# theislab/dca

Hardware: AMD Instinct MI355X
Metric: cells/sec training (ZINB AE, 68k x 20k) (higher is better)
Workload: dtype f32

## Files before the change

### dca_amd/csrc/dcahip_heads.hip

```cpp
#include <hip/hip_runtime.h>
#include <stdint.h>
#include <type_traits>
#include "dcahip.h"
#include "zinb_math.hpp"

namespace {

using f32x16 = __attribute__((ext_vector_type(16))) float;

constexpr int kTG = 32;
constexpr int kTR = 32;
constexpr int kLdS = 33;
constexpr int kWG = 2;
constexpr int kMaxGrid = 2048;
constexpr int kMaxSmallGrid = 8192;
constexpr int kCUs = 256;
constexpr int kZU = 4;
constexpr int kQCap = 320;

__device__ __forceinline__ int rowmap(int e, int hi) { return (e & 3) + 8 * (e >> 2) + 4 * hi; }

__device__ __forceinline__ void wave_sync() {
    __builtin_amdgcn_fence(__ATOMIC_RELEASE, "wavefront");
    __builtin_amdgcn_wave_barrier();
    __builtin_amdgcn_fence(__ATOMIC_ACQUIRE, "wavefront");
}

using f16x8 = __attribute__((ext_vector_type(8))) _Float16;
using f16x2v = __attribute__((ext_vector_type(2))) _Float16;
using f32x2v = __attribute__((ext_vector_type(2))) float;
using u32x4 = __attribute__((ext_vector_type(4))) unsigned;
using u32x2 = __attribute__((ext_vector_type(2))) unsigned;
using s16x4 = __attribute__((ext_vector_type(4))) short;

constexpr int kWR2 = 8;
constexpr int kWr8MinNT = 5;
constexpr int kHTile = 2 * 32 * 64;
constexpr int kTop = 13;
constexpr int kDExp0 = 8;
constexpr float kDLim = 30000.f;
constexpr int kDSlack = 2;
constexpr int kEHZero = 64;

#define MFMAH(a, b, c) __builtin_amdgcn_mfma_f32_32x32x16_f16(__builtin_bit_cast(f16x8, a), __builtin_bit_cast(f16x8, b), c, 0, 0, 0)

__device__ __forceinline__ unsigned pk_f16(float a, float b) {
    return __builtin_bit_cast(unsigned, __builtin_convertvector(f32x2v{a, b}, f16x2v));
}
__device__ __forceinline__ float resid_lo(unsigned p, float x) {
    float r;
    asm("v_fma_mix_f32 %0, %1, -1.0, %2 op_sel:[0,0,0] op_sel_hi:[1,0,0]" : "=v"(r) : "v"(p), "v"(x));
    return r;
}
__device__ __forceinline__ float resid_hi(unsigned p, float x) {
    float r;
    asm("v_fma_mix_f32 %0, %1, -1.0, %2 op_sel:[1,0,0] op_sel_hi:[1,0,0]" : "=v"(r) : "v"(p), "v"(x));
    return r;
}
__device__ __forceinline__ void split_pair(float x0, float x1, unsigned& p0, unsigned& p1) {
    p0 = pk_f16(x0, x1);
    p1 = pk_f16(resid_lo(p0, x0), resid_hi(p0, x1));
}
__device__ __forceinline__ void split8(const float (&x)[8], u32x4 (&f)[2]) {
#pragma unroll
    for (int j = 0; j < 4; ++j) {
        unsigned a, b;
        split_pair(x[2 * j], x[2 * j + 1], a, b);
        f[0][j] = a; f[1][j] = b;
    }
}
#ifdef DCA_EXP_H2_TWO
#define MFMA_H3(A, Bf, ACC) { ACC = MFMAH(A[0], Bf[1], ACC); ACC = MFMAH(A[0], Bf[0], ACC); }
#else
#define MFMA_H3(A, Bf, ACC) { ACC = MFMAH(A[1], Bf[0], ACC); ACC = MFMAH(A[0], Bf[1], ACC); ACC = MFMAH(A[0], Bf[0], ACC); }
#endif

__device__ __forceinline__ float pow2i(int e) { return __uint_as_float((unsigned)(127 + e) << 23); }
__device__ __forceinline__ int block_exp(float m) {
    if (!(m > 0.f) || !(m < INFINITY)) return 0;
    const int e = kTop + 1 - __builtin_amdgcn_frexp_expf(m);
    return e < -60 ? -60 : (e > 60 ? 60 : e);
}
__device__ __forceinline__ float wave_max(float v) {
    int l = (int)__builtin_amdgcn_mbcnt_hi(~0u, __builtin_amdgcn_mbcnt_lo(~0u, 0u));
    asm volatile("" : "+v"(l));
#pragma unroll
    for (int off = 32; off > 0; off >>= 1)
        v = fmaxf(v, __int_as_float(__builtin_amdgcn_ds_bpermute((l ^ off) << 2, __float_as_int(v))));
    return v;
}

struct HeadsArgs2 {
    const unsigned short* HA;
    const unsigned short* HT;
    const int* eH;
    const float* H; long ldh;
    float* gW; long ldg;
    float* g_theta;
    const float* Wh; long ldw;
    const float* bh;
    const float* theta_w;
    const float* y;  long ldy;
    const unsigned char* yc; long ldc;
    const int* ovf_ptr; const int* ovf_col; const float* ovf_val;
    const float* sf;
    const int* perm;
    const long long* cursor;
    float* ws_dw;  long dw_stride;
    float* ws_dh;
    int npart, nitems;
    const int* tile_order;
    double* partials;
    long plane, ldws;
    int B, hL, G;
    int S, NT;
    float ridge, inv_n;
    int d_exp;
    int tile_base;
};

__device__ __forceinline__ float escaped_count(const HeadsArgs2& p, long srow, int col) {
    float v = 255.f;
    if (p.ovf_ptr)
        for (int i = p.ovf_ptr[srow], e = p.ovf_ptr[srow + 1]; i < e; ++i)
            if (p.ovf_col[i] == col) { v = p.ovf_val[i]; break; }
    return v;
}

__global__ __launch_bounds__(256) void heads_split_h_kernel(const float* H, long ldh, int B, int hL,
                                                            unsigned short* HA, unsigned short* HT, int* eH) {
    __shared__ unsigned short tr[2][64][32 + 2];
    __shared__ float wm[4];
    const int t = blockIdx.x, tid = threadIdx.x;
    const int row = tid >> 3, k0 = (tid & 7) * 8;
    const long grow = (long)t * 32 + row;
    float x[8];
    float m = 0.f;
#pragma unroll
    for (int j = 0; j < 8; ++j) {
        x[j] = (grow < B && k0 + j < hL) ? H[grow * ldh + k0 + j] : 0.f;
        m = fmaxf(m, fabsf(x[j]));
    }
    m = wave_max(m);
    if ((tid & 63) == 0) wm[tid >> 6] = m;
    __syncthreads();
    const int e = block_exp(fmaxf(fmaxf(wm[0], wm[1]), fmaxf(wm[2], wm[3])));
    if (tid == 0) eH[t] = (fmaxf(fmaxf(wm[0], wm[1]), fmaxf(wm[2], wm[3])) > 0.f) ? e : kEHZero;
    const float sc = pow2i(e);
#pragma unroll
    for (int j = 0; j < 8; ++j) x[j] *= sc;
    u32x4 f[2];
    split8(x, f);
    const int pos = (row & 0x13) | ((row & 4) << 1) | ((row & 8) >> 1);
#pragma unroll
    for (int q = 0; q < 2; ++q) {
        *reinterpret_cast<u32x4*>(HA + (((long)t * 2 + q) * 32 + row) * 64 + k0) = f[q];
#pragma unroll
        for (int j = 0; j < 8; ++j) tr[q][k0 + j][pos] = (unsigned short)(f[q][j >> 1] >> (16 * (j & 1)));
    }
    __syncthreads();
    for (int c = tid; c < 2 * 64 * 4; c += 256) {
        const int q = c >> 8, i = (c >> 2) & 63, part = c & 3;
        u32x4 v;
#pragma unroll
        for (int j = 0; j < 4; ++j) v[j] = (unsigned)tr[q][i][part * 8 + 2 * j] | ((unsigned)tr[q][i][part * 8 + 2 * j + 1] << 16);
        *reinterpret_cast<u32x4*>(HT + (((long)t * 2 + q) * 64 + i) * 32 + part * 8) = v;
    }
}

template <bool HAS_PI, bool CONST_DISP, bool YC>
__global__ __launch_bounds__(64 * kWR2) void heads_fused_h2_kernel(HeadsArgs2 p) {
    using YV = std::conditional_t<YC, unsigned, float>;
    constexpr int WR = kWR2;
    constexpr int NH = 1 + (CONST_DISP ? 0 : 1) + (HAS_PI ? 1 : 0);
    constexpr int PI_H = NH - 1;
    constexpr int KT = 64;
    constexpr int ST_PLANE = kTG * kLdS;
    constexpr int QCAP = 192;
    constexpr int CELL_LD = 144;
    constexpr int HEAD_B = kTG * CELL_LD;
    constexpr int ROWT = 96;
    constexpr int PW_FLOATS = NH * HEAD_B / 4 + (CONST_DISP ? ST_PLANE : 0) + QCAP * 4 + ROWT;
    constexpr int NTHREADS = 64 * WR;
    constexpr int W_PIECE = 64 * 64;
    constexpr int W_FLOATS = NH * 2 * W_PIECE / 4;
    constexpr int NRED = NH * 2 * 16 + NH + 1;
    constexpr int BIAS_FLOATS = (NH + 1) * 32;
    constexpr int LDS_FLOATS = W_FLOATS + WR * PW_FLOATS + BIAS_FLOATS;
    static_assert((WR / 2) * NRED * 64 <= LDS_FLOATS, "dW reduce scratch");
    __shared__ __attribute__((aligned(16))) float lds[LDS_FLOATS];
    __shared__ double lred[WR];
    __shared__ float wmaxs[WR];

    const int tid = threadIdx.x, lane = tid & 63;
    const int wave = __builtin_amdgcn_readfirstlane(tid >> 6);
    const int l31 = lane & 31, hi = lane >> 5;
    const int r = wave;
    const long long cur = p.cursor ? *p.cursor : 0;
    double dacc = 0.0;
    bool first_item = true;
    const int s_wg = blockIdx.x % p.S, wq = blockIdx.x / p.S;
    const int ngb = p.nitems / p.S;
    const int full = ngb / p.npart, rem = ngb - full * p.npart;
    const int nrounds = full + ((rem > 0 && ((full & 1) ? p.npart - 1 - wq : wq) < rem) ? 1 : 0);
    const int kD0 = kDExp0 + p.d_exp;
    int eHmin = 1 << 20;
    for (int t = s_wg * WR + r; t < p.NT; t += p.S * WR) { const int e = p.eH[t]; eHmin = (e != kEHZero && e < eHmin) ? e : eHmin; }
    eHmin = __builtin_amdgcn_readfirstlane(eHmin == (1 << 20) ? 0 : eHmin);
#pragma unroll 1
    for (int j = 0; j < nrounds; ++j) {
    const int gb = j * p.npart + ((j & 1) ? p.npart - 1 - wq : wq);
    int s_opaque = s_wg;
    asm volatile("" : "+v"(s_opaque));
    const int s = __builtin_amdgcn_readfirstlane(s_opaque);
    const int gt = p.tile_order ? p.tile_order[gb + p.tile_base] : gb + p.tile_base;
    const int g0 = gt * kTG;
    const int gene = g0 + l31;
    const bool tile_ok = g0 < p.G;
    const bool gvalid = gene < p.G;

    unsigned char* const Wimg = reinterpret_cast<unsigned char*>(lds);
    unsigned char* const Pimg = reinterpret_cast<unsigned char*>(lds + W_FLOATS + wave * PW_FLOATS);
    float* const Th = lds + W_FLOATS + wave * PW_FLOATS + NH * HEAD_B / 4;
    u32x4* const Qe = reinterpret_cast<u32x4*>(lds + W_FLOATS + wave * PW_FLOATS + NH * HEAD_B / 4 + (CONST_DISP ? ST_PLANE : 0));
    float* const Bs = lds + W_FLOATS + WR * PW_FLOATS;
    int* const Rt = reinterpret_cast<int*>(lds + W_FLOATS + wave * PW_FLOATS + PW_FLOATS - ROWT);
    float* const Sft = reinterpret_cast<float*>(Rt + 64);

    int eW = 0;
    if (tile_ok) {
        constexpr int UNR = (NH * 64 * 8 + NTHREADS - 1) / NTHREADS;
        constexpr int ITEMS = NH * 64 * 8;
        float4 v[UNR];
        float m = 0.f;
#pragma unroll
        for (int u = 0; u < UNR; ++u) {
            const int idx = tid + u * NTHREADS;
            const int c4 = idx & 7, kq = (idx >> 3) & 63, h = (idx >> 9) < NH ? (idx >> 9) : NH - 1;
            const int kc = kq < p.hL ? kq : p.hL - 1;
            long gcol = g0 + c4 * 4;
            if (gcol > p.plane - 4) gcol = p.plane - 4;
            v[u] = *reinterpret_cast<const float4*>(p.Wh + (long)kc * p.ldw + (long)h * p.plane + gcol);
        }
#pragma unroll
        for (int u = 0; u < UNR; ++u) {
            const int idx = tid + u * NTHREADS;
            const int c4 = idx & 7, kq = (idx >> 3) & 63;
            const int gcol = g0 + c4 * 4;
            const bool kv = idx < ITEMS && kq < p.hL && gcol <= p.plane - 4;
            if (!kv || gcol + 0 >= p.G) v[u].x = 0.f;
            if (!kv || gcol + 1 >= p.G) v[u].y = 0.f;
            if (!kv || gcol + 2 >= p.G) v[u].z = 0.f;
            if (!kv || gcol + 3 >= p.G) v[u].w = 0.f;
            m = fmaxf(fmaxf(m, fmaxf(fabsf(v[u].x), fabsf(v[u].y))), fmaxf(fabsf(v[u].z), fabsf(v[u].w)));
        }
        m = wave_max(m);
        if (lane == 0) wmaxs[wave] = m;
        __syncthreads();
        m = fmaxf(fmaxf(fmaxf(wmaxs[0], wmaxs[1]), fmaxf(wmaxs[2], wmaxs[3])), fmaxf(fmaxf(wmaxs[4], wmaxs[5]), fmaxf(wmaxs[6], wmaxs[7])));
        eW = __builtin_amdgcn_readfirstlane(block_exp(m));
        const float wsc = pow2i(eW);
#pragma unroll
        for (int u = 0; u < UNR; ++u) {
            const int idx = tid + u * NTHREADS;
            if (idx >= ITEMS) continue;
            const int c4 = idx & 7, kq = (idx >> 3) & 63, h = idx >> 9;
            unsigned a0, a1, b0, b1;
            split_pair(v[u].x * wsc, v[u].y * wsc, a0, a1);
            split_pair(v[u].z * wsc, v[u].w * wsc, b0, b1);
            const int off = kq * 64 + ((((c4 >> 1) + (kq >> 2)) & 3) << 4) + ((c4 & 1) << 3);
            *reinterpret_cast<u32x2*>(Wimg + (h * 2 + 0) * W_PIECE + off) = u32x2{a0, b0};
            *reinterpret_cast<u32x2*>(Wimg + (h * 2 + 1) * W_PIECE + off) = u32x2{a1, b1};
        }
        if (tid < 32) {
            const bool gv = g0 + tid < p.G;
#pragma unroll
            for (int h = 0; h < NH; ++h) Bs[h * 32 + tid] = gv ? p.bh[(long)h * p.plane + g0 + tid] : 0.f;
            Bs[NH * 32 + tid] = (CONST_DISP && gv) ? p.theta_w[g0 + tid] : 0.f;
        }
    }
    __syncthreads();

    f32x16 dW[NH][2];
#pragma unroll
    for (int h = 0; h < NH; ++h)
#pragma unroll
        for (int ib = 0; ib < 2; ++ib)
#pragma unroll
            for (int e = 0; e < 16; ++e) dW[h][ib][e] = 0.f;
    float bsum[NH];
#pragma unroll
    for (int h = 0; h < NH; ++h) bsum[h] = 0.f;
    float thsum = 0.f;

    if (tile_ok) {
        const int gene_c = gvalid ? gene : p.G - 1;
        const float* const ycol = p.y + gene_c;
        const unsigned char* const ycolc = p.yc + gene_c;
        const unsigned ldy_u = YC ? (unsigned)p.ldc : (unsigned)p.ldy;
        auto count_at = [&](int sr) -> YV {
            if constexpr (YC) return (unsigned)ycolc[(unsigned long long)(unsigned)sr * ldy_u];
            else return ycol[(unsigned long long)(unsigned)sr * ldy_u];
        };
        const int tstep = p.S * WR;
        int t = s * WR + r;
        const long dh_tstride = (long)p.npart * (kTR * KT);
        float* const dh_part = p.ws_dh + (long)(blockIdx.x / p.S) * (kTR * KT);
        const int dh_lane = ((((l31 & 0x13) | ((l31 & 4) << 1) | ((l31 & 8) >> 1)) * KT) + 4 * hi) * 4;
        int srow_l = 0;
        float sf_l = 1.f;
        YV yA[kZU], yB[kZU];
        auto row_clamped = [&](int tt) { const int rl = tt * kTR + l31; return rl < p.B ? rl : p.B - 1; };
        auto load_srow = [&](int tt) { const int rlc = row_clamped(tt); return p.perm ? p.perm[cur + rlc] : (int)(cur + rlc); };
        const __amdgpu_buffer_rsrc_t ha_rs = __builtin_amdgcn_make_buffer_rsrc(
            const_cast<unsigned short*>(p.HA), 0, p.NT * (kHTile * 2), 0x00020000);
        const __amdgpu_buffer_rsrc_t ht_rs = __builtin_amdgcn_make_buffer_rsrc(
            const_cast<unsigned short*>(p.HT), 0, p.NT * (kHTile * 2), 0x00020000);
        const int ha_lane = l31 * 128 + hi * 64;
        const int ht_lane = l31 * 64 + hi * 16;
        u32x4 ha0[2];
        auto load_ha = [&](int tt, int ks, u32x4 (&dst)[2]) {
            const int so = tt * (kHTile * 2);
            int ha_o = ha_lane;
            asm volatile("" : "+v"(ha_o));
#pragma unroll
            for (int q = 0; q < 2; ++q)
                dst[q] = __builtin_bit_cast(u32x4, __builtin_amdgcn_raw_buffer_load_b128(ha_rs, ha_o + q * 4096 + ks * 16, so, 0));
        };
        auto load_ht = [&](int tt, int ks, u32x4 (&dst)[2][2]) {
            const int so = tt * (kHTile * 2);
            int ht_o = ht_lane;
            asm volatile("" : "+v"(ht_o));
#pragma unroll
            for (int q = 0; q < 2; ++q)
#pragma unroll
                for (int ib = 0; ib < 2; ++ib)
                    dst[q][ib] = __builtin_bit_cast(u32x4, __builtin_amdgcn_raw_buffer_load_b128(
                        ht_rs, ht_o + q * 4096 + ib * 2048 + ks * 32, so, 0));
        };
        const int t16 = lane & 15, c8 = 4 * ((lane >> 4) & 1) + (t16 & 3);
        int wtr[4];
#pragma unroll
        for (int rr = 0; rr < 4; ++rr)
            wtr[rr] = hi * 2048 + (t16 >> 2) * 64 + ((((c8 >> 1) + rr) & 3) << 4) + ((c8 & 1) << 3);
        int wdr[2];
#pragma unroll
        for (int gs = 0; gs < 2; ++gs) wdr[gs] = l31 * 64 + (((2 * gs + hi + (l31 >> 2)) & 3) << 4);
        auto w_tr = [&](int h, int q, int ks) {
            const unsigned char* b0 = Wimg + (h * 2 + q) * W_PIECE + ks * 512;
            const s16x4 lo = __builtin_amdgcn_ds_read_tr16_b64_v4i16(
                (__attribute__((address_space(3))) s16x4*)(b0 + wtr[(2 * ks) & 3]));
            const s16x4 hi4 = __builtin_amdgcn_ds_read_tr16_b64_v4i16(
                (__attribute__((address_space(3))) s16x4*)(b0 + 256 + wtr[(2 * ks + 1) & 3]));
            u32x4 o;
            const u32x2 a = __builtin_bit_cast(u32x2, lo), b = __builtin_bit_cast(u32x2, hi4);
            o[0] = a[0]; o[1] = a[1]; o[2] = b[0]; o[3] = b[1];
            return o;
        };
        auto w_dr = [&](int h, int q, int jb, int gs) {
            return *reinterpret_cast<const u32x4*>(Wimg + (h * 2 + q) * W_PIECE + jb * 2048 + wdr[gs]);
        };
        const int cell_lane = l31 * CELL_LD + 2 * hi * 16;
        const int dtr = (8 * hi + (t16 >> 2)) * CELL_LD + c8 * 16;

        int eHt = 0;
        if (t < p.NT) {
            srow_l = load_srow(t);
            sf_l = p.sf[srow_l];
            eHt = p.eH[t];
            load_ha(t, 0, ha0);
            if (lane < 32) { Rt[l31] = srow_l; Sft[l31] = sf_l; }
            wave_sync();
            {
                const int4 r4 = *reinterpret_cast<const int4*>(Rt + 4 * hi);
                yA[0] = count_at(r4.x); yA[1] = count_at(r4.y); yA[2] = count_at(r4.z); yA[3] = count_at(r4.w);
            }
        }
        int rb = 0;
        int accE = eHmin + kD0;
        int tile_no = wave >> 2;
        for (; t < p.NT; t += tstep) {
            if ((tile_no++) & 1) __builtin_amdgcn_s_setprio(1); else __builtin_amdgcn_s_setprio(0);
            const int row0 = t * kTR;
            const int tn = t + tstep < p.NT ? t + tstep : t;
            eHt = __builtin_amdgcn_readfirstlane(eHt);
            const bool hzero = eHt == kEHZero;
            if (hzero) eHt = 0;
            const int kDa = accE - eHt;
            const int kDt = (!hzero && kDa <= kD0 && kDa >= kD0 - kDSlack) ? kDa : kD0;
            const float fscale = pow2i(eHt + eW), funscale = pow2i(-(eHt + eW));
            int kDe = kDt;
            float lacc;
            const float thw = CONST_DISP ? Bs[NH * 32 + l31] : 0.f;
            const int srow_n = load_srow(tn);
            if (lane < 32) Rt[(rb ^ 1) * 32 + l31] = srow_n;
            const int eHn = p.eH[tn];
            float scs = 0.f;
            int qn = 0;
            float dmax = 0.f;
            auto z_sparse = [&](int q0, int cnt) {
                const bool act = lane < cnt;
                const u32x4 ent = Qe[q0 + (act ? lane : 0)];
                const unsigned e = ent[0];
                const int gq = (e >> 5) & 31, row = e & 31;
                const float sfr = __shfl(sf_l, row, 64);
                const int sr = __shfl(srow_l, row, 64);
                const float am = __uint_as_float(ent[1]);
                const float ad = CONST_DISP ? Bs[NH * 32 + gq] : __uint_as_float(ent[2]);
                const float ap = HAS_PI ? __uint_as_float(ent[3]) : 0.f;
                float yq = (float)(e >> 16);
                if (__ballot(act && (e >> 16) == 0xFFFFu)) {
                    if (act && (e >> 16) == 0xFFFFu) yq = YC ? escaped_count(p, sr, g0 + gq) : p.y[(long)sr * p.ldy + g0 + gq];
                    __builtin_amdgcn_s_waitcnt(0x0F70);
                }
                float o[3] = {0.f, 0.f, 0.f};
                float nll;
                if (HAS_PI) {
                    nll = zinb_nz_elem<CONST_DISP, YC>(am, ad, ap, sfr, yq, p.ridge, o[0], o[1], o[2]);
                } else {
                    float dmu = 0.f, dth = 0.f, dpi = 0.f;
                    const Heads hd = head_acts<HAS_PI, CONST_DISP>(am, ad, ap, sfr);
                    nll = nll_elem<HAS_PI, true, true, YC>(hd, yq, p.ridge, dmu, dth, dpi);
                    o[0] = dmu * hd.gm; o[1] = dth * hd.gd;
                }
                lacc += act ? nll : 0.f;
                o[0] *= scs; o[1] *= scs; o[2] *= scs;
                dmax = fmaxf(dmax, act ? fmaxf(fmaxf(fabsf(o[0]), CONST_DISP ? 0.f : fabsf(o[1])), fabsf(o[2])) : 0.f);
                if (act) {
                    const int pos = (row & 0x13) | ((row & 4) << 1) | ((row & 8) >> 1);
                    unsigned char* pa = Pimg + gq * CELL_LD + (pos >> 2) * 16 + (pos & 3) * 2;
                    auto put = [&](int h, float v) {
                        const _Float16 h1 = (_Float16)v;
                        const _Float16 h2 = (_Float16)(v - (float)h1);
                        *reinterpret_cast<_Float16*>(pa + h * HEAD_B) = h1;
                        *reinterpret_cast<_Float16*>(pa + h * HEAD_B + 8) = h2;
                    };
                    put(0, o[0]);
                    if (CONST_DISP) Th[gq * kLdS + row] = o[1]; else put(1, o[1]);
                    if (HAS_PI) put(PI_H, o[2]);
                }
            };
            auto z_flush = [&](bool last) {
                while (qn >= 64 || (last && qn > 0)) {
                    const int c = qn < 64 ? qn : 64;
                    wave_sync();
                    z_sparse(qn - c, c);
                    qn -= c;
                }
            };
            auto z_dense = [&](auto fullv, int grp, const YV (&yv)[kZU]) {
                constexpr bool FULLV = decltype(fullv)::value;
                unsigned char* const cell = Pimg + cell_lane + ((grp & 1) + 4 * (grp >> 1)) * 16;
                float i_am[kZU], i_ad[kZU], i_ap[kZU];
                {
                    const float4 vm = *reinterpret_cast<const float4*>(cell);
                    i_am[0] = vm.x; i_am[1] = vm.y; i_am[2] = vm.z; i_am[3] = vm.w;
                    if (CONST_DISP) {
#pragma unroll
                        for (int j = 0; j < kZU; ++j) i_ad[j] = thw;
                    } else {
                        const float4 vd = *reinterpret_cast<const float4*>(cell + HEAD_B);
                        i_ad[0] = vd.x; i_ad[1] = vd.y; i_ad[2] = vd.z; i_ad[3] = vd.w;
                    }
                    if (HAS_PI) {
                        const float4 vp = *reinterpret_cast<const float4*>(cell + PI_H * HEAD_B);
                        i_ap[0] = vp.x; i_ap[1] = vp.y; i_ap[2] = vp.z; i_ap[3] = vp.w;
                    } else {
#pragma unroll
                        for (int j = 0; j < kZU; ++j) i_ap[j] = 0.f;
                    }
                }
                float o_m[kZU], o_d[kZU], o_p[kZU];
                bool o_nz[kZU];
                const float4 sf4 = *reinterpret_cast<const float4*>(Sft + 8 * grp + 4 * hi);
                const float sfj[kZU] = {sf4.x, sf4.y, sf4.z, sf4.w};
#pragma unroll
                for (int j = 0; j < kZU; ++j) {
                    const int row = rowmap(grp * kZU + j, hi);
                    const bool valid = FULLV || ((row0 + row < p.B) && gvalid);
                    const YV yj = yv[j];
                    bool nz;
                    if constexpr (YC) nz = valid && yj != 0u;
                    else nz = valid && (HAS_PI ? !(yj < kZeroThresh) : (yj != 0.f));
                    const float sc = (valid && !nz) ? scs : 0.f;
                    if (HAS_PI) {
                        float gmv, gdv, gpv;
                        const float nll = zinb_zero_elem<CONST_DISP>(i_am[j], i_ad[j], i_ap[j], sfj[j], p.ridge, gmv, gdv, gpv);
                        lacc += (valid && !nz) ? nll : 0.f;
                        o_m[j] = gmv * sc;
                        o_d[j] = gdv * sc;
                        o_p[j] = gpv * sc;
                        dmax = fmaxf(dmax, fmaxf(fabsf(o_m[j]), fabsf(o_p[j])));
                    } else {
                        float gmv, gdv;
                        const float nll = nb_zero_elem<CONST_DISP>(i_am[j], i_ad[j], sfj[j], gmv, gdv);
                        lacc += (valid && !nz) ? nll : 0.f;
                        o_m[j] = gmv * sc;
                        o_d[j] = gdv * sc;
                        o_p[j] = 0.f;
                        dmax = fmaxf(dmax, fabsf(o_m[j]));
                    }
                    if (!CONST_DISP) dmax = fmaxf(dmax, fabsf(o_d[j]));
                    o_nz[j] = nz;
                }
                {
                    auto put4 = [&](int h, const float (&v)[kZU]) {
                        unsigned a0, a1, b0, b1;
                        split_pair(v[0], v[1], a0, a1);
                        split_pair(v[2], v[3], b0, b1);
                        *reinterpret_cast<u32x4*>(cell + h * HEAD_B) = u32x4{a0, b0, a1, b1};
                    };
                    put4(0, o_m);
                    if (!CONST_DISP) put4(1, o_d);
                    if (HAS_PI) put4(PI_H, o_p);
                }
#pragma unroll
                for (int j = 0; j < kZU; ++j) {
                    const int row = rowmap(grp * kZU + j, hi);
                    const bool nz = o_nz[j];
                    const unsigned long long m = __ballot(nz);
                    const int slot = qn + __builtin_amdgcn_mbcnt_hi((unsigned)(m >> 32), __builtin_amdgcn_mbcnt_lo((unsigned)m, 0u));
                    if (nz) {
                        const YV yj = yv[j];
                        unsigned y16;
                        if constexpr (YC) y16 = yj == 255u ? 0xFFFFu : yj;
                        else y16 = (yj < 65535.f && yj == floorf(yj)) ? (unsigned)yj : 0xFFFFu;
                        Qe[slot] = u32x4{(unsigned)(l31 * 32 + row) | (y16 << 16), __float_as_uint(i_am[j]), __float_as_uint(i_ad[j]),
                                         __float_as_uint(i_ap[j])};
                    } else if (CONST_DISP) {
                        Th[l31 * kLdS + row] = o_d[j];
                    }
                    qn += __popcll(m);
                    if (j == 1) z_flush(false);
                }
                z_flush(false);
            };
            auto load_y = [&](int half, int grp, YV (&yv)[kZU]) {
                const int4 r4 = *reinterpret_cast<const int4*>(Rt + (rb ^ half) * 32 + 8 * grp + 4 * hi);
                yv[0] = count_at(r4.x); yv[1] = count_at(r4.y); yv[2] = count_at(r4.z); yv[3] = count_at(r4.w);
            };
            u32x4 htb[2][2][2];
            auto z_loop = [&](auto fullv) {
#pragma unroll 1
                for (int grp = 0; grp < 16 / kZU; ++grp) {
                    if (grp + 1 < 16 / kZU) load_y(0, grp + 1, yB);
                    else load_y(1, 0, yB);
                    z_dense(fullv, grp, yA);
#pragma unroll
                    for (int j = 0; j < kZU; ++j) yA[j] = yB[j];
                }
                load_ht(t, 0, htb[0]);
                __builtin_amdgcn_sched_barrier(0);
                z_flush(true);
            };
            for (;;) {
            f32x16 acc[NH];
#pragma unroll
            for (int h = 0; h < NH; ++h) {
                const float bias_h = Bs[h * 32 + l31] * fscale;
#pragma unroll
                for (int e = 0; e < 16; ++e) acc[h][e] = bias_h;
            }
            {
                u32x4 hb[2][2];
#pragma unroll
                for (int q = 0; q < 2; ++q) hb[0][q] = ha0[q];
#pragma unroll
                for (int ks = 0; ks < 4; ++ks) {
                    if (ks < 3) load_ha(t, ks + 1, hb[(ks + 1) & 1]);
                    __builtin_amdgcn_sched_barrier(0);
#pragma unroll
                    for (int h = 0; h < NH; ++h) {
                        u32x4 bf[2] = {w_tr(h, 0, ks), w_tr(h, 1, ks)};
                        MFMA_H3(hb[ks & 1], bf, acc[h])
                    }
                }
            }
#pragma unroll
            for (int h = 0; h < NH; ++h)
#pragma unroll
                for (int g = 0; g < 4; ++g)
                    *reinterpret_cast<float4*>(Pimg + h * HEAD_B + cell_lane + ((g & 1) + 4 * (g >> 1)) * 16) =
                        make_float4(acc[h][4 * g] * funscale, acc[h][4 * g + 1] * funscale, acc[h][4 * g + 2] * funscale, acc[h][4 * g + 3] * funscale);
            wave_sync();

            scs = pow2i(kDe);
            lacc = 0.f;
            qn = 0;
            dmax = 0.f;
            if (row0 + kTR <= p.B && g0 + kTG <= p.G) z_loop(std::true_type{}); else z_loop(std::false_type{});
            if (!__ballot(!(dmax <= kDLim))) break;
            const float mx = wave_max(dmax);
            const int need = __builtin_amdgcn_readfirstlane(__builtin_amdgcn_frexp_expf(mx) - 1 - kTop);
            if (!(need > 0) || kDe < kDt - 200) break;
            kDe -= need > 100 ? 100 : need;
            load_y(0, 0, yA);
            load_ha(t, 0, ha0);
            wave_sync();
            }
            dacc += (double)lacc;
            const float sf_n = p.sf[srow_n];
            wave_sync();
            if (!hzero && accE != eHt + kDe) {
                const int mv = eHt + kDe - accE;
                accE = eHt + kDe;
#pragma unroll
                for (int h = 0; h < NH; ++h)
#pragma unroll
                    for (int ib = 0; ib < 2; ++ib)
#pragma unroll
                        for (int e = 0; e < 16; ++e) dW[h][ib][e] = __builtin_amdgcn_ldexpf(dW[h][ib][e], mv);
            }

            const __amdgpu_buffer_rsrc_t dh_rs = __builtin_amdgcn_make_buffer_rsrc(
                dh_part + (long)t * dh_tstride, 0, kTR * KT * 4, 0x00020000);
            const __amdgpu_buffer_rsrc_t dh_rq = __builtin_amdgcn_make_buffer_rsrc(
                dh_part + (long)t * dh_tstride, 0, first_item ? 0 : kTR * KT * 4, 0x00020000);
            f32x16 dHa[2];
            int dh_o = dh_lane;
            asm volatile("" : "+v"(dh_o));
            load_ht(t, 1, htb[1]);
#pragma unroll
            for (int jb = 0; jb < 2; ++jb)
#pragma unroll
                for (int eq = 0; eq < 4; ++eq) {
                    const u32x4 u = __builtin_bit_cast(u32x4, __builtin_amdgcn_raw_buffer_load_b128(dh_rq, dh_o + 128 * jb + 32 * eq, 0, 0));
#pragma unroll
                    for (int w = 0; w < 4; ++w) { const unsigned uw = u[w]; dHa[jb][4 * eq + w] = __uint_as_float(uw); }
                }
            __builtin_amdgcn_sched_barrier(0);
            float tsum[NH];
#pragma unroll
            for (int h = 0; h < NH; ++h) tsum[h] = 0.f;
#pragma unroll
            for (int ks = 0; ks < 2; ++ks)
#pragma unroll
                for (int h = 0; h < NH; ++h) {
                    u32x4 bf[2];
#pragma unroll
                    for (int q = 0; q < 2; ++q) {
                        const unsigned char* c0 = Pimg + h * HEAD_B + cell_lane + 4 * ks * 16 + 8 * q;
                        const u32x2 lo = *reinterpret_cast<const u32x2*>(c0), hi2 = *reinterpret_cast<const u32x2*>(c0 + 16);
                        bf[q] = u32x4{lo[0], lo[1], hi2[0], hi2[1]};
#pragma unroll
                        for (int w = 0; w < 4; ++w) {
                            const unsigned pw = bf[q][w];
                            tsum[h] = __builtin_amdgcn_fdot2(__builtin_bit_cast(f16x2v, pw), f16x2v{(_Float16)1.f, (_Float16)1.f}, tsum[h], false);
                        }
                    }
#pragma unroll
                    for (int ib = 0; ib < 2; ++ib) {
                        u32x4 af[2] = {htb[ks][0][ib], htb[ks][1][ib]};
                        MFMA_H3(af, bf, dW[h][ib])
                    }
                }
#pragma unroll
            for (int h = 0; h < NH; ++h) asm volatile("" : "+v"(tsum[h]));
            {
                const float gun = pow2i(-kDe);
#pragma unroll
                for (int h = 0; h < NH; ++h) bsum[h] = fmaf(tsum[h], gun, bsum[h]);
                if (CONST_DISP) {
                    float ts = 0.f;
#pragma unroll
                    for (int e = 0; e < 16; ++e) ts += Th[l31 * kLdS + rowmap(e, hi)];
                    thsum = fmaf(ts, gun, thsum);
                }
            }
            load_ha(tn, 0, ha0);
            __builtin_amdgcn_sched_barrier(0);
            {
                const float fs = pow2i(kDe + eW), fu = pow2i(-(kDe + eW));
#pragma unroll
                for (int jb = 0; jb < 2; ++jb)
#pragma unroll
                    for (int e = 0; e < 16; ++e) {
                        float x = dHa[jb][e];
                        asm("v_mul_f32 %0, %1, %0" : "+v"(x) : "s"(fs));
                        dHa[jb][e] = x;
                    }
#pragma unroll
                for (int h = 0; h < NH; ++h)
#pragma unroll
                    for (int gs = 0; gs < 2; ++gs) {
                        u32x4 af[2];
#pragma unroll
                        for (int q = 0; q < 2; ++q) {
                            const unsigned char* b0 = Pimg + h * HEAD_B + gs * 16 * CELL_LD + 8 * q + dtr;
                            const s16x4 lo = __builtin_amdgcn_ds_read_tr16_b64_v4i16((__attribute__((address_space(3))) s16x4*)(b0));
                            const s16x4 hi4 = __builtin_amdgcn_ds_read_tr16_b64_v4i16((__attribute__((address_space(3))) s16x4*)(b0 + 4 * CELL_LD));
                            const u32x2 a = __builtin_bit_cast(u32x2, lo), b = __builtin_bit_cast(u32x2, hi4);
                            af[q] = u32x4{a[0], a[1], b[0], b[1]};
                        }
#pragma unroll
                        for (int jb = 0; jb < 2; ++jb) {
                            u32x4 bf[2] = {w_dr(h, 0, jb, gs), w_dr(h, 1, jb, gs)};
                            MFMA_H3(bf, af, dHa[jb])
                        }
                    }
#pragma unroll
                for (int jb = 0; jb < 2; ++jb)
#pragma unroll
                    for (int eq = 0; eq < 4; ++eq) {
                        u32x4 v;
#pragma unroll
                        for (int w = 0; w < 4; ++w) v[w] = __float_as_uint(dHa[jb][4 * eq + w] * fu);
                        __builtin_amdgcn_raw_buffer_store_b128(v, dh_rs, dh_o + 128 * jb + 32 * eq, 0, 0);
                    }
            }
            srow_l = srow_n;
            sf_l = sf_n;
            eHt = eHn;
            if (lane < 32) Sft[l31] = sf_n;
            rb ^= 1;
            wave_sync();
        }
        {
#pragma unroll
            for (int h = 0; h < NH; ++h)
#pragma unroll
                for (int ib = 0; ib < 2; ++ib)
#pragma unroll
                    for (int e = 0; e < 16; ++e) dW[h][ib][e] = __builtin_amdgcn_ldexpf(dW[h][ib][e], -accE);
        }
    }

    __syncthreads();

    {
        float* red = lds;
#pragma unroll
        for (int step = 1; step < WR; step *= 2) {
            const int slot = r / (2 * step);
            float* rs = red + (long)slot * NRED * 64 + lane;
            if (r % (2 * step) == step) {
                int n = 0;
#pragma unroll
                for (int h = 0; h < NH; ++h)
#pragma unroll
                    for (int ib = 0; ib < 2; ++ib)
#pragma unroll
                        for (int e = 0; e < 16; ++e) rs[(n++) * 64] = dW[h][ib][e];
#pragma unroll
                for (int h = 0; h < NH; ++h) rs[(n++) * 64] = bsum[h];
                rs[(n++) * 64] = thsum;
            }
            __syncthreads();
            if (r % (2 * step) == 0 && r + step < WR) {
                int n = 0;
#pragma unroll
                for (int h = 0; h < NH; ++h)
#pragma unroll
                    for (int ib = 0; ib < 2; ++ib)
#pragma unroll
                        for (int e = 0; e < 16; ++e) dW[h][ib][e] += rs[(n++) * 64];
#pragma unroll
                for (int h = 0; h < NH; ++h) bsum[h] += rs[(n++) * 64];
                thsum += rs[(n++) * 64];
            }
            __syncthreads();
        }
    }
    if (r == 0 && tile_ok) {
        const bool direct = p.S == 1;
        float* out = direct ? p.gW : p.ws_dw + (long)s * p.dw_stride;
        const long ldo = direct ? p.ldg : p.ldws;
        const float fin = direct ? p.inv_n : 1.f;
        const bool cw = gene < p.plane;
#pragma unroll
        for (int h = 0; h < NH; ++h) {
#pragma unroll
            for (int ib = 0; ib < 2; ++ib)
#pragma unroll
                for (int e = 0; e < 16; ++e) {
                    const int i = ib * 32 + rowmap(e, hi);
                    if (cw && i < p.hL) out[(long)i * ldo + (long)h * p.plane + gene] = dW[h][ib][e] * fin;
                }
            const float bv = bsum[h] + __shfl_xor(bsum[h], 32, 64);
            if (cw && hi == 0) out[(long)p.hL * ldo + (long)h * p.plane + gene] = bv * fin;
        }
        if (CONST_DISP) {
            const float tv = thsum + __shfl_xor(thsum, 32, 64);
            if (direct) {
                if (gvalid && hi == 0) {
                    const float e = expf(p.theta_w[gene]);
                    p.g_theta[gene] = (e >= 1e-3f && e <= 1e4f) ? tv * p.inv_n * e : 0.f;
                }
            } else if (cw && hi == 0) {
                out[(long)(p.hL + 1) * ldo + gene] = tv;
            }
        }
    }
    __syncthreads();
    first_item = false;
    }

#pragma unroll
    for (int off = 32; off > 0; off >>= 1) dacc += __shfl_down(dacc, off, 64);
    if (lane == 0) lred[wave] = dacc;
    __syncthreads();
    if (tid == 0) {
        double v = 0.0;
        for (int w = 0; w < WR; ++w) v += lred[w];
        p.partials[blockIdx.x] = v;
    }
}


struct ReduceDwArgs {
    const float* ws; int S; long stride; int hL; long ldws, ncols; float* gW; long ldg;
    const float* theta_w; float* g_theta; int G;
    float scale;
    const float* ws2; int S2; const int* tail_tiles; int ntail; long plane;
    int tail_first;
};

__device__ __forceinline__ void reduce_dw_body(const ReduceDwArgs& q, int bid, int nblk) {
    const int hL = q.hL;
    const long ldws = q.ldws, ncols = q.ncols; float* gW = q.gW; const long ldg = q.ldg;
    const float* theta_w = q.theta_w; float* g_theta = q.g_theta; const int G = q.G;
    const float sc = q.scale;
    __shared__ unsigned tailbm[kMaxGrid / 32];
    if (q.ntail > 0) {
        for (int i = threadIdx.x; i < kMaxGrid / 32; i += 256) tailbm[i] = 0u;
        __syncthreads();
        for (int i = threadIdx.x; i < q.ntail; i += 256) {
            const int tl = q.tail_tiles ? q.tail_tiles[i] : q.tail_first + i;
            if (tl >= 0 && tl < kMaxGrid) atomicOr(&tailbm[tl >> 5], 1u << (tl & 31));
        }
        __syncthreads();
    }
    auto is_tail = [&](long col_in_plane) { const int tl = (int)(col_in_plane / kTG); return q.ntail > 0 && ((tailbm[tl >> 5] >> (tl & 31)) & 1u); };
    if ((ncols & 3) == 0 && (ldws & 3) == 0 && (ldg & 3) == 0 && (q.stride & 3) == 0 && (q.plane & 3) == 0 &&
        ((reinterpret_cast<uintptr_t>(q.ws) | reinterpret_cast<uintptr_t>(gW) | reinterpret_cast<uintptr_t>(q.ws2)) & 15) == 0) {
        const long nq = ncols >> 2, totalq = (long)(hL + 1) * nq;
        for (long idx = (long)bid * 256 + threadIdx.x; idx < totalq; idx += (long)nblk * 256) {
            const long i = idx / nq, c = (idx - i * nq) << 2;
            const bool tl = is_tail(c % q.plane);
            const float* ws = tl ? q.ws2 : q.ws; const int S = tl ? q.S2 : q.S; const long stride = q.stride;
            float4 v = *reinterpret_cast<const float4*>(ws + i * ldws + c);
            for (int s = 1; s < S; ++s) {
                const float4 x = *reinterpret_cast<const float4*>(ws + (long)s * stride + i * ldws + c);
                v.x += x.x; v.y += x.y; v.z += x.z; v.w += x.w;
            }
            v.x *= sc; v.y *= sc; v.z *= sc; v.w *= sc;
            *reinterpret_cast<float4*>(gW + i * ldg + c) = v;
        }
    } else {
        const long total = (long)(hL + 1) * ncols;
        for (long idx = (long)bid * 256 + threadIdx.x; idx < total; idx += (long)nblk * 256) {
            const long i = idx / ncols, c = idx - i * ncols;
            const bool tl = is_tail(c % q.plane);
            const float* ws = tl ? q.ws2 : q.ws; const int S = tl ? q.S2 : q.S;
            float v = 0.f;
            for (int s = 0; s < S; ++s) v += ws[(long)s * q.stride + i * ldws + c];
            gW[i * ldg + c] = v * sc;
        }
    }
    if (g_theta) {
        for (long c = (long)bid * 256 + threadIdx.x; c < G; c += (long)nblk * 256) {
            const bool tl = is_tail(c);
            const float* ws = tl ? q.ws2 : q.ws; const int S = tl ? q.S2 : q.S; const long stride = q.stride;
            float v = 0.f;
            for (int s = 0; s < S; ++s) v += ws[(long)s * stride + (long)(hL + 1) * ldws + c];
            const float e = expf(theta_w[c]);
            g_theta[c] = (e >= 1e-3f && e <= 1e4f) ? v * sc * e : 0.f;
        }
    }
}

__global__ __launch_bounds__(256) void heads_reduce_dw_kernel(ReduceDwArgs q) { reduce_dw_body(q, blockIdx.x, gridDim.x); }

struct ReduceDhArgs {
    const float* ws; int ntg, B, Bpad, KT, hL; float* dH; long lddh; float scale;
    const double* loss_partials; int n_partials; double loss_scale; float* loss_out;
    const float* ws2; int ntg2;
};

template <int GL>
__device__ __forceinline__ void reduce_dh_body(const ReduceDhArgs& q, int bid) {
    const float* ws = q.ws; const int ntg = q.ntg, B = q.B, KT = q.KT, hL = q.hL; float* dH = q.dH; const long lddh = q.lddh;
    const double* loss_partials = q.loss_partials; const int n_partials = q.n_partials; const double loss_scale = q.loss_scale;
    float* loss_out = q.loss_out;
    constexpr int OUT = 256 / GL;
    __shared__ float4 red[256];
    const int o = threadIdx.x % OUT, gl = threadIdx.x / OUT;
    const int q4 = KT / 4;
    const long nq = (long)B * q4;
    const long quad = (long)bid * OUT + o;
    float4 v = make_float4(0.f, 0.f, 0.f, 0.f);
    if (quad < nq) {
        const long tq = (long)kTR * q4;
        const long t = quad / tq, within = quad - t * tq;
        const float4* src = reinterpret_cast<const float4*>(ws) + t * ntg * tq + within;
        for (int gt0 = gl; gt0 < ntg; gt0 += 8 * GL) {
            float4 x[8];
#pragma unroll
            for (int u = 0; u < 8; ++u) {
                const int gt = gt0 + u * GL;
                x[u] = src[(long)(gt < ntg ? gt : gl) * tq];
            }
#pragma unroll
            for (int u = 0; u < 8; ++u)
                if (gt0 + u * GL < ntg) { v.x += x[u].x; v.y += x[u].y; v.z += x[u].z; v.w += x[u].w; }
        }
        if (q.ntg2 > 0) {
            const float4* src2 = reinterpret_cast<const float4*>(q.ws2) + t * q.ntg2 * tq + within;
            for (int gt = gl; gt < q.ntg2; gt += GL) { const float4 x = src2[(long)gt * tq]; v.x += x.x; v.y += x.y; v.z += x.z; v.w += x.w; }
        }
    }
    red[threadIdx.x] = v;
    __syncthreads();
    if (gl == 0 && quad < nq) {
#pragma unroll
        for (int k = 1; k < GL; ++k) {
            const float4 x = red[k * OUT + o];
            v.x += x.x; v.y += x.y; v.z += x.z; v.w += x.w;
        }
        const long row = quad / q4;
        const int i = (int)(quad - row * q4) * 4;
        float* d = dH + row * lddh + i;
        if (i + 0 < hL) d[0] = v.x * q.scale;
        if (i + 1 < hL) d[1] = v.y * q.scale;
        if (i + 2 < hL) d[2] = v.z * q.scale;
        if (i + 3 < hL) d[3] = v.w * q.scale;
    }
    if (loss_out && bid == 0) {
        __shared__ double lsum[256];
        double a = 0.0;
        for (int i = threadIdx.x; i < n_partials; i += 256) a += loss_partials[i];
        lsum[threadIdx.x] = a;
        __syncthreads();
        for (int st = 128; st > 0; st >>= 1) {
            if ((int)threadIdx.x < st) lsum[threadIdx.x] += lsum[threadIdx.x + st];
            __syncthreads();
        }
        if (threadIdx.x == 0) {
            float lf = (float)(lsum[0] * loss_scale);
            if (isnan(lf)) lf = INFINITY;
            *loss_out = lf;
        }
    }
}

template <int GL>
__global__ __launch_bounds__(256) void heads_reduce_dh_kernel(ReduceDhArgs q) { reduce_dh_body<GL>(q, blockIdx.x); }

template <int GL>
__global__ __launch_bounds__(256) void heads_reduce_both_kernel(ReduceDhArgs qh, ReduceDwArgs qw, int n_dh) {
    if ((int)blockIdx.x < n_dh) reduce_dh_body<GL>(qh, blockIdx.x);
    else reduce_dw_body(qw, blockIdx.x - n_dh, gridDim.x - n_dh);
}


struct HeadsPlan {
    bool small;
    int HLB, WR, S, NT, ntg, ngb, grid;
    int nitems, npart;
    long ldws, dw_stride, dw_bytes, dh_bytes, hs_bytes;
    int nmain, ntail, S2, grid2, npart2, nitems2;
    long dh2_bytes, dw2_bytes;
};

inline bool al16(const void* p) { return (reinterpret_cast<uintptr_t>(p) & 15) == 0; }

bool make_heads_plan(int B, int hL, int G, long plane, int flags, HeadsPlan* out) {
    if (flags & (DCAHIP_NLL_POISSON | DCAHIP_NLL_MSE)) return false;
    if (B <= 0 || G <= 0 || hL <= 0 || hL > 64 || plane < G || (plane & 3) || plane > ((G + 31) & ~31)) return false;
    if (B > (1 << 22)) return false;
    const bool has_pi = flags & DCAHIP_NLL_HAS_PI, cdisp = flags & DCAHIP_NLL_CONST_DISP;
    const int NH = 1 + (cdisp ? 0 : 1) + (has_pi ? 1 : 0);
    HeadsPlan p;
    p.HLB = 2;
    p.NT = (B + kTR - 1) / kTR;
    p.ntg = (G + kTG - 1) / kTG;
    p.ngb = p.ntg;
    if (p.ngb > kMaxGrid) return false;
    p.small = p.NT < kWr8MinNT;
    static_assert((kWr8MinNT - 1) * kMaxGrid <= kMaxSmallGrid, "loss partials of the four-wave kernel");
    p.WR = p.small ? 1 : kWR2;
    const int smax = (p.NT + p.WR - 1) / p.WR;
    double best = 1e300;
    p.S = 1;
    const double item_cost = 0.75;
    for (int S = 1; S <= smax && (long)S * p.ngb <= kMaxGrid; ++S) {
        const long items = (long)S * p.ngb;
        const long rounds = (items + kCUs - 1) / kCUs;
        const int tiles = (p.NT + S * p.WR - 1) / (S * p.WR);
        const double cost = (double)rounds * (tiles + item_cost);
        if (cost < best - 1e-9) { best = cost; p.S = S; }
    }
    p.nitems = p.S * p.ngb;
    p.grid = p.nitems;
    p.npart = p.ntg;
    if (p.small) {
        p.S = p.NT;
        p.nitems = p.NT * p.ntg;
        p.grid = p.nitems;
        p.npart = p.ntg;
    } else {
        const int res = kCUs / p.S * p.S;
        if (p.grid > res) p.grid = res;
        p.npart = p.grid / p.S;
    }
    p.nmain = p.ngb; p.ntail = 0; p.S2 = 0; p.grid2 = 0; p.npart2 = 0; p.nitems2 = 0;
    if (!p.small && p.S >= 2) {
        const int full = p.ngb / p.npart, rem = p.ngb - full * p.npart;
        const int tiles = (p.NT + p.S * p.WR - 1) / (p.S * p.WR);
        if (full >= 1 && rem > 0) {
            const double uniform = (double)(full + 1) * (tiles + item_cost);
            double best2 = 1e300; int bestS = 0;
            for (int S2 = 2 * p.S; S2 <= smax && (long)S2 * rem <= kMaxGrid; S2 *= 2) {
                const long items2 = (long)S2 * rem;
                const long rounds2 = (items2 + kCUs - 1) / kCUs;
                const int tiles2 = (p.NT + S2 * p.WR - 1) / (S2 * p.WR);
                const double c2 = (double)rounds2 * (tiles2 + item_cost);
                if (c2 < best2 - 1e-9) { best2 = c2; bestS = S2; }
            }
            if (bestS && (double)full * (tiles + item_cost) + best2 + 1.0 < uniform - 0.5) {
// ... 577 lines not shown
```

Before: 4.582 million.

## Overlap per-item prologue loads with weight-tile staging and carry across rounds

Hoists the first row-tile prologue (perm row index, eH exponent, size factor, HA fragment, first count gather) ahead of the weight-tile staging, so its global-load latency overlaps the W load, quantize and LDS write. On later gene-tile rounds it reuses data already prefetched at the end of the previous round, by wrapping the next-tile index back to t0 and tracking this with a `carried` flag. Bias and theta loads move into registers early. In z_loop, the row-index LDS reads are prefetched one group ahead. This raises register pressure and adds subtle state-carry logic across rounds, including the Rt buffer parity.

After: 4.639 million, median of 6. 1.2% higher.

```diff
diff --git a/dca_amd/csrc/dcahip_heads.hip b/dca_amd/csrc/dcahip_heads.hip
--- a/dca_amd/csrc/dcahip_heads.hip
+++ b/dca_amd/csrc/dcahip_heads.hip
@@ -207,6 +207,11 @@
     int eHmin = 1 << 20;
     for (int t = s_wg * WR + r; t < p.NT; t += p.S * WR) { const int e = p.eH[t]; eHmin = (e != kEHZero && e < eHmin) ? e : eHmin; }
     eHmin = __builtin_amdgcn_readfirstlane(eHmin == (1 << 20) ? 0 : eHmin);
+    int srow_l = 0;
+    float sf_l = 1.f;
+    int eHt = 0;
+    u32x4 ha0[2] = {};
+    bool carried = false;
 #pragma unroll 1
     for (int j = 0; j < nrounds; ++j) {
     const int gb = j * p.npart + ((j & 1) ? p.npart - 1 - wq : wq);
@@ -227,24 +232,67 @@
     int* const Rt = reinterpret_cast<int*>(lds + W_FLOATS + wave * PW_FLOATS + PW_FLOATS - ROWT);
     float* const Sft = reinterpret_cast<float*>(Rt + 64);
 
+    const int gene_c = gvalid ? gene : p.G - 1;
+    const float* const ycol = p.y + gene_c;
+    const unsigned char* const ycolc = p.yc + gene_c;
+    const unsigned ldy_u = YC ? (unsigned)p.ldc : (unsigned)p.ldy;
+    auto count_at = [&](int sr) -> YV {
+        if constexpr (YC) return (unsigned)ycolc[(unsigned long long)(unsigned)sr * ldy_u];
+        else return ycol[(unsigned long long)(unsigned)sr * ldy_u];
+    };
+    YV yA[kZU], yB[kZU];
+    auto row_clamped = [&](int tt) { const int rl = tt * kTR + l31; return rl < p.B ? rl : p.B - 1; };
+    auto load_srow = [&](int tt) { const int rlc = row_clamped(tt); return p.perm ? p.perm[cur + rlc] : (int)(cur + rlc); };
+    const __amdgpu_buffer_rsrc_t ha_rs = __builtin_amdgcn_make_buffer_rsrc(
+        const_cast<unsigned short*>(p.HA), 0, p.NT * (kHTile * 2), 0x00020000);
+    const int ha_lane = l31 * 128 + hi * 64;
+    auto load_ha = [&](int tt, int ks, u32x4 (&dst)[2]) {
+        const int so = tt * (kHTile * 2);
+        int ha_o = ha_lane;
+        asm volatile("" : "+v"(ha_o));
+#pragma unroll
+        for (int q = 0; q < 2; ++q)
+            dst[q] = __builtin_bit_cast(u32x4, __builtin_amdgcn_raw_buffer_load_b128(ha_rs, ha_o + q * 4096 + ks * 16, so, 0));
+    };
+    const int t0 = s * WR + r;
+    if (tile_ok && t0 < p.NT && !carried) {
+        srow_l = load_srow(t0);
+        eHt = p.eH[t0];
+        sf_l = p.sf[srow_l];
+        load_ha(t0, 0, ha0);
+    }
+    auto item_head = [&]() {
+        if (lane < 32) Rt[l31] = srow_l;
+        wave_sync();
+        const int4 r4 = *reinterpret_cast<const int4*>(Rt + 4 * hi);
+        yA[0] = count_at(r4.x); yA[1] = count_at(r4.y); yA[2] = count_at(r4.z); yA[3] = count_at(r4.w);
+    };
+
     int eW = 0;
     if (tile_ok) {
         constexpr int UNR = (NH * 64 * 8 + NTHREADS - 1) / NTHREADS;
         constexpr int ITEMS = NH * 64 * 8;
         float4 v[UNR];
+        int tidp = tid;
+        asm volatile("" : "+v"(tidp));
         float m = 0.f;
 #pragma unroll
         for (int u = 0; u < UNR; ++u) {
-            const int idx = tid + u * NTHREADS;
+            const int idx = tidp + u * NTHREADS;
             const int c4 = idx & 7, kq = (idx >> 3) & 63, h = (idx >> 9) < NH ? (idx >> 9) : NH - 1;
             const int kc = kq < p.hL ? kq : p.hL - 1;
             long gcol = g0 + c4 * 4;
             if (gcol > p.plane - 4) gcol = p.plane - 4;
             v[u] = *reinterpret_cast<const float4*>(p.Wh + (long)kc * p.ldw + (long)h * p.plane + gcol);
         }
+        float bv[NH + 1];
+#pragma unroll
+        for (int h = 0; h < NH; ++h) bv[h] = p.bh[(long)h * p.plane + gene_c];
+        bv[NH] = CONST_DISP ? p.theta_w[gene_c] : 0.f;
+        item_head();
 #pragma unroll
         for (int u = 0; u < UNR; ++u) {
-            const int idx = tid + u * NTHREADS;
+            const int idx = tidp + u * NTHREADS;
             const int c4 = idx & 7, kq = (idx >> 3) & 63;
             const int gcol = g0 + c4 * 4;
             const bool kv = idx < ITEMS && kq < p.hL && gcol <= p.plane - 4;
@@ -262,7 +310,7 @@
         const float wsc = pow2i(eW);
 #pragma unroll
         for (int u = 0; u < UNR; ++u) {
-            const int idx = tid + u * NTHREADS;
+            const int idx = tidp + u * NTHREADS;
             if (idx >= ITEMS) continue;
             const int c4 = idx & 7, kq = (idx >> 3) & 63, h = idx >> 9;
             unsigned a0, a1, b0, b1;
@@ -273,10 +321,9 @@
             *reinterpret_cast<u32x2*>(Wimg + (h * 2 + 1) * W_PIECE + off) = u32x2{a1, b1};
         }
         if (tid < 32) {
-            const bool gv = g0 + tid < p.G;
-#pragma unroll
-            for (int h = 0; h < NH; ++h) Bs[h * 32 + tid] = gv ? p.bh[(long)h * p.plane + g0 + tid] : 0.f;
-            Bs[NH * 32 + tid] = (CONST_DISP && gv) ? p.theta_w[g0 + tid] : 0.f;
+#pragma unroll
+            for (int h = 0; h < NH; ++h) Bs[h * 32 + tid] = gvalid ? bv[h] : 0.f;
+            Bs[NH * 32 + tid] = (CONST_DISP && gvalid) ? bv[NH] : 0.f;
         }
     }
     __syncthreads();
@@ -294,39 +341,14 @@
     float thsum = 0.f;
 
     if (tile_ok) {
-        const int gene_c = gvalid ? gene : p.G - 1;
-        const float* const ycol = p.y + gene_c;
-        const unsigned char* const ycolc = p.yc + gene_c;
-        const unsigned ldy_u = YC ? (unsigned)p.ldc : (unsigned)p.ldy;
-        auto count_at = [&](int sr) -> YV {
-            if constexpr (YC) return (unsigned)ycolc[(unsigned long long)(unsigned)sr * ldy_u];
-            else return ycol[(unsigned long long)(unsigned)sr * ldy_u];
-        };
         const int tstep = p.S * WR;
-        int t = s * WR + r;
+        int t = t0;
         const long dh_tstride = (long)p.npart * (kTR * KT);
         float* const dh_part = p.ws_dh + (long)(blockIdx.x / p.S) * (kTR * KT);
         const int dh_lane = ((((l31 & 0x13) | ((l31 & 4) << 1) | ((l31 & 8) >> 1)) * KT) + 4 * hi) * 4;
-        int srow_l = 0;
-        float sf_l = 1.f;
-        YV yA[kZU], yB[kZU];
-        auto row_clamped = [&](int tt) { const int rl = tt * kTR + l31; return rl < p.B ? rl : p.B - 1; };
-        auto load_srow = [&](int tt) { const int rlc = row_clamped(tt); return p.perm ? p.perm[cur + rlc] : (int)(cur + rlc); };
-        const __amdgpu_buffer_rsrc_t ha_rs = __builtin_amdgcn_make_buffer_rsrc(
-            const_cast<unsigned short*>(p.HA), 0, p.NT * (kHTile * 2), 0x00020000);
         const __amdgpu_buffer_rsrc_t ht_rs = __builtin_amdgcn_make_buffer_rsrc(
             const_cast<unsigned short*>(p.HT), 0, p.NT * (kHTile * 2), 0x00020000);
-        const int ha_lane = l31 * 128 + hi * 64;
         const int ht_lane = l31 * 64 + hi * 16;
-        u32x4 ha0[2];
-        auto load_ha = [&](int tt, int ks, u32x4 (&dst)[2]) {
-            const int so = tt * (kHTile * 2);
-            int ha_o = ha_lane;
-            asm volatile("" : "+v"(ha_o));
-#pragma unroll
-            for (int q = 0; q < 2; ++q)
-                dst[q] = __builtin_bit_cast(u32x4, __builtin_amdgcn_raw_buffer_load_b128(ha_rs, ha_o + q * 4096 + ks * 16, so, 0));
-        };
         auto load_ht = [&](int tt, int ks, u32x4 (&dst)[2][2]) {
             const int so = tt * (kHTile * 2);
             int ht_o = ht_lane;
@@ -363,26 +385,14 @@
         const int cell_lane = l31 * CELL_LD + 2 * hi * 16;
         const int dtr = (8 * hi + (t16 >> 2)) * CELL_LD + c8 * 16;
 
-        int eHt = 0;
-        if (t < p.NT) {
-            srow_l = load_srow(t);
-            sf_l = p.sf[srow_l];
-            eHt = p.eH[t];
-            load_ha(t, 0, ha0);
-            if (lane < 32) { Rt[l31] = srow_l; Sft[l31] = sf_l; }
-            wave_sync();
-            {
-                const int4 r4 = *reinterpret_cast<const int4*>(Rt + 4 * hi);
-                yA[0] = count_at(r4.x); yA[1] = count_at(r4.y); yA[2] = count_at(r4.z); yA[3] = count_at(r4.w);
-            }
-        }
+        if (t < p.NT && lane < 32) Sft[l31] = sf_l;
         int rb = 0;
         int accE = eHmin + kD0;
         int tile_no = wave >> 2;
         for (; t < p.NT; t += tstep) {
             if ((tile_no++) & 1) __builtin_amdgcn_s_setprio(1); else __builtin_amdgcn_s_setprio(0);
             const int row0 = t * kTR;
-            const int tn = t + tstep < p.NT ? t + tstep : t;
+            const int tn = t + tstep < p.NT ? t + tstep : t0;
             eHt = __builtin_amdgcn_readfirstlane(eHt);
             const bool hzero = eHt == kEHZero;
             if (hzero) eHt = 0;
@@ -541,10 +551,12 @@
             };
             u32x4 htb[2][2][2];
             auto z_loop = [&](auto fullv) {
+                int4 rn = *reinterpret_cast<const int4*>(Rt + rb * 32 + 8 + 4 * hi);
 #pragma unroll 1
                 for (int grp = 0; grp < 16 / kZU; ++grp) {
-                    if (grp + 1 < 16 / kZU) load_y(0, grp + 1, yB);
-                    else load_y(1, 0, yB);
+                    yB[0] = count_at(rn.x); yB[1] = count_at(rn.y); yB[2] = count_at(rn.z); yB[3] = count_at(rn.w);
+                    const int g2 = grp + 2;
+                    rn = *reinterpret_cast<const int4*>(Rt + (g2 < 16 / kZU ? rb * 32 + 8 * g2 : (rb ^ 1) * 32 + 8 * (g2 - 16 / kZU)) + 4 * hi);
                     z_dense(fullv, grp, yA);
 #pragma unroll
                     for (int j = 0; j < kZU; ++j) yA[j] = yB[j];
@@ -715,6 +727,7 @@
             rb ^= 1;
             wave_sync();
         }
+        carried = carried || t0 < p.NT;
         {
 #pragma unroll
             for (int h = 0; h < NH; ++h)
```
